# Kari-Genomics-Lab/iDeLUCS

Measured on AMD Instinct MI355X. Metric: sequences/sec (k-mer vectorise + 1 epoch), k=6 batch 512, higher is better.
Workload: dtype f32

## Files before the change

idelucs_amd/csrc/scaler_device.h:

```cpp
#pragma once
#include <hip/hip_runtime.h>
#include <stdint.h>

#include "planes.h"
#include "store_policy.h"

namespace idl_dev {

__device__ __forceinline__ float std_f32(float x, double m, double s)
{
    const float t = (float)((double)x - m);
    return (float)((double)t / s);
}

__device__ __forceinline__ float std_f32_rcp(float x, double m, double s, double r)
{
    const double t = (double)(float)((double)x - m);
    const double q = t * r;
    return (float)fma(fma(-q, s, t), r, q);
}

struct GatherArgs {
    const float *feats;
    int64_t n, f, view_stride;
    const int64_t *pair_idx;
    const int64_t *base;
    int64_t batch, n_pairs;
    const double *mean, *scale, *inv_scale;
    float *y;
    int64_t base_add;
    uint16_t *yh, *yl;
    int *over;
    int wt;
};

__device__ __forceinline__ void gather_row(const GatherArgs &g, int64_t row, int tid, int nthreads)
{
    const int64_t b = row < g.batch ? row : row - g.batch;
    const int64_t at = (g.base ? *g.base : 0) + g.base_add + b;
    if (g.n_pairs >= 0 && at >= g.n_pairs) return;
    const int64_t pair = g.pair_idx[at];
    const int64_t m = pair / g.n, s = pair - m * g.n;
    const float *src = g.feats + (row < g.batch ? 0 : (m + 1) * g.view_stride) + s * g.f;
    float *dst = g.y + row * g.f;
    if ((g.f & 3) == 0) {
        const float4 *src4 = (const float4 *)src;
        float4 *dst4 = (float4 *)dst;
        const int64_t n4 = g.f / 4;
        for (int64_t i0 = tid; i0 < n4; i0 += 4 * (int64_t)nthreads) {
            float4 vv[4];
#pragma unroll
            for (int u = 0; u < 4; ++u) {
                const int64_t i = i0 + (int64_t)u * nthreads;
                if (i < n4) vv[u] = src4[i];
            }
#pragma unroll
// ... 16 lines not shown
                }
                dst4[i] = o;
            }
        }
    } else {
        for (int64_t i = tid; i < g.f; i += nthreads) dst[i] = std_f32(src[i], g.mean[i], g.scale[i]);
    }
}

constexpr int GATHER_ROWS = 8;

__host__ __device__ inline int64_t gather_blocks(int64_t f, int64_t batch)
{
    if (f & 3) return 2 * batch;
    return ((2 * batch + GATHER_ROWS - 1) / GATHER_ROWS) * ((f / 4 + 255) / 256);
}

template <int R>
__host__ __device__ inline int64_t gather_tiles(int64_t f, int64_t batch)
{
    return ((2 * batch + R - 1) / R) * ((f / 4 + 255) / 256);
}

template <int R>
__device__ __forceinline__ void gather_tile(const GatherArgs &g, int64_t blk, int tid)
{
    const int64_t n4 = g.f / 4, slices = (n4 + 255) / 256;
    const int64_t rg = blk / slices, i = (blk - rg * slices) * 256 + tid;
    if (i >= n4) return;
    const int64_t base = (g.base ? *g.base : 0) + g.base_add;
    const bool wt = (g.wt & idl_store::WT_NEXT_PLANES) != 0;
    const bool paired = wt && (n4 & 1) == 0 && ((((uintptr_t)g.yh) | ((uintptr_t)g.yl)) & 15u) == 0;
    const float4 *src4[R];
    float4 vv[R];
#pragma unroll
    for (int u = 0; u < R; ++u) {
        const int64_t row = rg * R + u;
        const int64_t b = row < g.batch ? row : row - g.batch;
        const int64_t at = base + b;
        src4[u] = nullptr;
        if (row < 2 * g.batch && (g.n_pairs < 0 || at < g.n_pairs)) {
            const int64_t pair = g.pair_idx[at];
            const int64_t m = pair / g.n, s = pair - m * g.n;
            src4[u] = (const float4 *)(g.feats + (row < g.batch ? 0 : (m + 1) * g.view_stride) + s * g.f);
        }
    }
#pragma unroll
    for (int u = 0; u < R; ++u)
        if (src4[u] != nullptr) vv[u] = src4[u][i];
    const int64_t c = i * 4;
    double mu[4], sc[4], rc[4];
#pragma unroll
    for (int e = 0; e < 4; ++e) { mu[e] = g.mean[c + e]; sc[e] = g.scale[c + e]; rc[e] = g.inv_scale ? g.inv_scale[c + e] : 0.0; }
#pragma unroll
    for (int u = 0; u < R; ++u) {
        if (src4[u] == nullptr) continue;
        const float4 v = vv[u];
        float4 o;
        if (g.inv_scale != nullptr) {
            o.x = std_f32_rcp(v.x, mu[0], sc[0], rc[0]); o.y = std_f32_rcp(v.y, mu[1], sc[1], rc[1]);
            o.z = std_f32_rcp(v.z, mu[2], sc[2], rc[2]); o.w = std_f32_rcp(v.w, mu[3], sc[3], rc[3]);
        } else {
            o.x = std_f32(v.x, mu[0], sc[0]); o.y = std_f32(v.y, mu[1], sc[1]);
            o.z = std_f32(v.z, mu[2], sc[2]); o.w = std_f32(v.w, mu[3], sc[3]);
        }
        if (g.y != nullptr) idl_store::store16((float4 *)(g.y + (rg * R + u) * g.f) + i, o, wt);
        if (g.yh != nullptr) {
            constexpr float ps = (float)(1 << idl_planes::X_EXP);
            uint2 h, l;
            if (idl_planes::split4(o.x * ps, o.y * ps, o.z * ps, o.w * ps, h, l) && g.over != nullptr) *g.over = 1;
            if (paired) {
                const bool odd = (tid & 1) != 0;
                idl_store::store16_wt((uint2 *)((odd ? g.yl : g.yh) + (rg * R + u) * g.f) + (i - (odd ? 1 : 0)), idl_store::pair_planes(h, l, odd));
            } else {
                ((uint2 *)(g.yh + (rg * R + u) * g.f))[i] = h;
                ((uint2 *)(g.yl + (rg * R + u) * g.f))[i] = l;
            }
        }
    }
}

__device__ __forceinline__ void gather_block(const GatherArgs &g, int64_t blk, int tid)
{
    if (g.f & 3) { gather_row(g, blk, tid, 256); return; }
    gather_tile<GATHER_ROWS>(g, blk, tid);
}

}
```

idelucs_amd/csrc/train_step.hip:

```cpp
#include <stdlib.h>
#include "dev_env.h"
#include <string.h>

#include "common.h"
#include "iic_device.h"
#include "nce_device.h"
#include "scaler_device.h"
#include "wave_ops.h"
#include "wgrad_device.h"
#include "l1_device.h"
#include "l1_planes_device.h"
#include "wgrad_planes_device.h"
#include "mid_fwd_device.h"

namespace {

using mid_dev::H1;
using mid_dev::H2;
using mid_dev::MAX_CPL;
using mid_dev::f32x4_t;
constexpr int COL_PARTS = 64;


#ifdef IDL_PHASE_STAMPS
// ... 30 lines not shown
        if (c < C) {
            float acc = b3[c];
            const float *wr = W3 + (int64_t)c * H2;
#pragma unroll 8
            for (int h = 0; h < H2; ++h) acc = fmaf(sh[h], wr[h], acc);
            lg.v[t] = acc;
        }
    }
    mid_dev::softmax_row(lg, row, lane, C, true, z);
    __builtin_amdgcn_wave_barrier();
}

__global__ __launch_bounds__(256) void head_fwd_kernel(const float *lat, const float *W3, const float *b3, int m, int C, int train,
                                                       uint64_t seed, const int64_t *ctl, float *f, float *inv, float *r2, float *z)
{
    __shared__ float sh[4][H2];
    const int w = threadIdx.x >> 6, lane = threadIdx.x & 63;
    const int row = blockIdx.x * 4 + w;
    if (row >= m) return;
    head_row(lat[(int64_t)row * H2 + lane], row, lane, sh[w], W3, b3, C, train, seed, (uint32_t)ctl[0], f, inv, r2, z);
}

constexpr int MID_WAVES = mid_dev::WAVES;
constexpr int MID_GATHER_ROWS = 4;

template <bool TIN>
__device__ __forceinline__ void mid_fwd_body(float *__restrict__ a1, const float *__restrict__ b1, const float *__restrict__ W2,
                                                                  const float *__restrict__ b2, const float *__restrict__ W3,
                                                                  const float *__restrict__ b3, int m, int C, int train, uint64_t seed,
                                                                  const int64_t *__restrict__ ctl, float *__restrict__ f,
                                                                  float *__restrict__ inv, float *__restrict__ r2, float *__restrict__ z,
                                                                  int n_rows_wg, int tile0, int tile1, const idl_dev::GatherArgs &gth, const int bid)
{
    if (bid >= n_rows_wg) {
        const int blk = tile0 + (bid - n_rows_wg) * 4 + (int)(threadIdx.x >> 8);
        if (blk < tile1) idl_dev::gather_tile<MID_GATHER_ROWS>(gth, (int64_t)blk, (int)(threadIdx.x & 255));
        return;
    }
    __shared__ float part[MID_WAVES][16][H2];
    float (*R2t)[H2 + 4] = (float (*)[H2 + 4])&part[0][0][0];
    float (*LG)[64 * MAX_CPL + 1] = (float (*)[64 * MAX_CPL + 1])&part[2][0][0];
    const int lane = threadIdx.x & 63, wv = threadIdx.x >> 6, l = lane & 15, q = lane >> 4;
    const int r0 = bid * 16;
    uint64_t *stf = IDL_PHASE_BUF(1, bid);
    IDL_PHASE_STAMP(stf, 0);
    const int k0 = 32 * wv + 8 * q;
    float4 *src = (float4 *)(a1 + (int64_t)(r0 + l) * H1 + k0);
    float *srcT = a1 + (int64_t)k0 * m + r0 + l;
    float4 av[2] = {make_float4(0.f, 0.f, 0.f, 0.f), make_float4(0.f, 0.f, 0.f, 0.f)};
    float4 bb[2] = {make_float4(0.f, 0.f, 0.f, 0.f), make_float4(0.f, 0.f, 0.f, 0.f)};
    mid_dev::W2Tile bw[4];
    auto load_bw = [&]() {
#pragma unroll
        for (int ct = 0; ct < 4; ++ct) bw[ct] = mid_dev::load_w2(W2, ct, l, k0);
    };
    float t8[8] = {0.f, 0.f, 0.f, 0.f, 0.f, 0.f, 0.f, 0.f};
    if (TIN) {
#pragma unroll
        for (int i = 0; i < 8; ++i) t8[i] = srcT[(int64_t)i * m];
        av[0] = make_float4(t8[0], t8[1], t8[2], t8[3]); av[1] = make_float4(t8[4], t8[5], t8[6], t8[7]);
    } else {
        av[0] = src[0]; av[1] = src[1];
// ... 328 lines not shown
            acc += v;
        }
    }
    sh[w][lane] = acc;
    __syncthreads();
    if (w == 0 && c < n) job.partial[(int64_t)blockIdx.y * n + c] = (sh[0][lane] + sh[1][lane]) + (sh[2][lane] + sh[3][lane]);
}

struct MidBwdArgs {
    const float *z, *r2, *f, *inv, *G, *dP0, *W3, *W2, *act1;
    float *dlogits, *dlat, *dr1, *partial1, *partial2, *partial3, *dW3_part;
    int64_t *ctl; int64_t batch_advance;
    int g_parts, m, C, train; float nce_coef;
    int act1_t;
    uint16_t *dr1h, *dr1l;
    int *dscale, *dover;
    const float *dzs;
};

template <bool BIG = false, bool DP = false>
__device__ __forceinline__ void mid_bwd_body(const MidBwdArgs &a, int tile0, int tile1, const idl_dev::GatherArgs &gth, const int bid)
{
    extern __shared__ float mid_dyn[];
    if (bid >= COL_PARTS) {
        const int blk = tile0 + (bid - COL_PARTS) * 4 + (int)(threadIdx.x >> 8);
        if (blk < tile1) idl_dev::gather_tile<MID_GATHER_ROWS>(gth, (int64_t)blk, (int)(threadIdx.x & 255));
        return;
    }
    __shared__ float DL[16][H2 + 4];
    __shared__ float R2s[16][H2];
    __shared__ float DLG[16][64 * MAX_CPL];
    __shared__ float shz[MID_WAVES][64 * MAX_CPL];
    __shared__ float sP[48 * 48], sW3[48 * H2];
    const int lane = threadIdx.x & 63, wv = threadIdx.x >> 6, l = lane & 15, q = lane >> 4, tid = threadIdx.x;
    const int m = a.m, C = a.C, B = m / 2;
    constexpr bool small = !BIG;
    const int rows = (m + COL_PARTS - 1) / COL_PARTS;
    const int r0 = bid * rows;
    const int r1 = (r0 + rows < m) ? r0 + rows : m;
    uint64_t *stb = IDL_PHASE_BUF(2, bid);
    IDL_PHASE_STAMP(stb, 0);
    if (a.ctl != nullptr && bid == 0 && tid == 0) a.ctl[1] += a.batch_advance;
    __shared__ unsigned int s_dmx, s_dcnt;
    const int dk = DP ? a.dscale[1] : 0;
    if (DP && tid == 0) { s_dmx = 0u; s_dcnt = 0u; }
    unsigned int dmx = 0u;
    if (small) {
        for (int i = tid; i < C * C; i += 64 * MID_WAVES) sP[i] = a.dP0[i];
        for (int i = tid; i < C * H2; i += 64 * MID_WAVES) sW3[i] = a.W3[i];
    } else {
        for (int i = tid; i < C * H2; i += 64 * MID_WAVES) mid_dyn[i] = a.W3[i];
    }
    float bw[2][16];
#pragma unroll
    for (int s = 0; s < 16; ++s) {
// ... 209 lines not shown
    }
    if (te < H2) a.partial2[(int64_t)bid * H2 + te] = s23;
    else if (te < H2 + C) a.partial3[(int64_t)bid * C + te - H2] = s23;
    if (a.dW3_part != nullptr) {
#pragma unroll
        for (int i = 0; i < 3; ++i) {
            const int o = te + 1024 * i;
            if (o < C * H2) a.dW3_part[(int64_t)bid * C * H2 + o] = acc3[i];
        }
    }
    IDL_PHASE_STAMP(stb, 6);
}
struct MidBwdParams { MidBwdArgs a; int tile0, tile1; idl_dev::GatherArgs gth; };
static_assert(sizeof(MidBwdParams) + idl::PLAN_PARAMS <= idl::PLAN_BYTES, "MidBwdParams does not fit a plan record");

template <bool BIG = false, bool DP = false>
__global__ __launch_bounds__(64 * MID_WAVES) void mid_bwd_kernel(MidBwdArgs a, int tile0, int tile1, idl_dev::GatherArgs gth)
{
    mid_bwd_body<BIG, DP>(a, tile0, tile1, gth, (int)blockIdx.x);
}

__global__ __launch_bounds__(64 * MID_WAVES) void mid_bwd_batched_kernel(const unsigned char *__restrict__ plans)
{
    const MidBwdParams &p = *(const MidBwdParams *)(plans + (size_t)blockIdx.x * idl::PLAN_BYTES + idl::PLAN_PARAMS);
    if (p.a.dr1h != nullptr) mid_bwd_body<false, true>(p.a, p.tile0, p.tile1, p.gth, (int)blockIdx.y);
    else mid_bwd_body<false, false>(p.a, p.tile0, p.tile1, p.gth, (int)blockIdx.y);
}

__global__ __launch_bounds__(64 * MID_WAVES) void mid_bwd_big_batched_kernel(const unsigned char *__restrict__ plans)
{
    const MidBwdParams &p = *(const MidBwdParams *)(plans + (size_t)blockIdx.x * idl::PLAN_BYTES + idl::PLAN_PARAMS);
    mid_bwd_body<true, true>(p.a, p.tile0, p.tile1, p.gth, (int)blockIdx.y);
}

struct RmsArgs {
    const float *loss_rows;
    float *out;
    int loss_m;
    float w_nce, w_iic;
    float *p[8];
    const float *g[8];
    float *v[8];
    int64_t n[8];
    int parts[8];
    int count;
    const float *wg_dy, *wg_x; float *wg_grad;
// ... 232 lines not shown
#pragma unroll
        for (int u = 0; u < RED_U; ++u) {
            const int64_t i = i0 + 256 * u < r.slab4 ? i0 + 256 * u : r.slab4 - 1;
#pragma unroll
            for (int p = 0; p < l1p_dev::KSPLIT; ++p) v[u][p] = r.part[(int64_t)p * r.slab4 + i];
        }
#pragma unroll
        for (int u = 0; u < RED_U; ++u) {
            float4 acc = v[u][0];
#pragma unroll
            for (int p = 1; p < l1p_dev::KSPLIT; ++p) { acc.x += v[u][p].x; acc.y += v[u][p].y; acc.z += v[u][p].z; acc.w += v[u][p].w; }
            if (i0 + 256 * u < r.slab4) r.part[i0 + 256 * u] = acc;
        }
        return;
    }
    if (with_tail) rmsprop_body<true>(a, hyper, ctl, batch_advance, 0, 0, idl_dev::GatherArgs{}, (int)blockIdx.x, (int)threadIdx.x);
}

struct SumsFwdArgs {
    const float *b1, *W2, *b2, *W3, *b3; float *r1T; int m, C, train; uint64_t seed; float *f, *inv, *r2, *z; int tile0, tile1; idl_dev::GatherArgs gth;
};
constexpr int SUMS_FWD_ROWS = 8;
constexpr int SUMS_FWD_LDS = (MID_WAVES * SUMS_FWD_ROWS * H2 + 16 * (H2 + 4) + SUMS_FWD_ROWS * (64 * MAX_CPL + 1)) * (int)sizeof(float);

__device__ __forceinline__ void sums_fwd_body(const ReduceArgs &r, const SumsFwdArgs &p, float *smem, const int bid)
{
    constexpr int ROWS = SUMS_FWD_ROWS, GROUPS = 16 / ROWS, SPL = l1p_dev::KSPLIT / GROUPS, Q0 = 4 - ROWS / 4;
    if (bid >= r.blocks) {
        const int blk = p.tile0 + (bid - r.blocks) * 4 + (int)(threadIdx.x >> 8);
        if (blk < p.tile1) idl_dev::gather_tile<MID_GATHER_ROWS>(p.gth, (int64_t)blk, (int)(threadIdx.x & 255));
        return;
    }
    float (*ps)[ROWS][H2] = (float (*)[ROWS][H2])smem;
    float (*R2t)[H2 + 4] = (float (*)[H2 + 4])(smem + MID_WAVES * ROWS * H2);
    float (*LG)[64 * MAX_CPL + 1] = (float (*)[64 * MAX_CPL + 1])(smem + MID_WAVES * ROWS * H2 + 16 * (H2 + 4));
    const int lane = threadIdx.x & 63, wv = threadIdx.x >> 6, l = lane & 15, q = lane >> 4;
    const int grp = l / ROWS, rr = l % ROWS;
    const bool own = grp == GROUPS - 1;
    const int m = p.m, C = p.C, train = p.train;
    const int r0 = bid * ROWS;
    const int k0 = 32 * wv + 8 * q;
    const int64_t e4 = ((int64_t)(r0 + rr) * H1 + k0) / 4;
    float4 pv[SPL][2];
#pragma unroll
    for (int j = 0; j < SPL; ++j) {
        const float4 *src = r.part + (int64_t)(SPL * grp + j) * r.slab4 + e4;
        pv[j][0] = src[0]; pv[j][1] = src[1];
    }
    float4 bb[2];
    bb[0] = *(const float4 *)(p.b1 + k0); bb[1] = *(const float4 *)(p.b1 + k0 + 4);
    mid_dev::W2Tile bw[4];
#pragma unroll
    for (int ct = 0; ct < 4; ++ct) bw[ct] = mid_dev::load_w2(p.W2, ct, l, k0);
// ... 195 lines not shown
                 float *f, float *inv, float *r2, float *z, void *stream)
{
    IDL_REQUIRE(lat && W3 && b3 && ctl && f && inv && r2 && z, "NULL buffer");
    IDL_REQUIRE(m >= 1 && C >= 1 && C <= 64 * MAX_CPL, "head_fwd: n_clusters must be in 1..256");
    hipLaunchKernelGGL(head_fwd_kernel, dim3((unsigned)((m + 3) / 4)), dim3(256), 0, (hipStream_t)stream, lat, W3, b3, m, C, train, seed,
                       ctl, f, inv, r2, z);
    IDL_HIP_TRY(hipGetLastError());
    return IDL_OK;
}

int idl_mid_fwd(float *a1, const float *W2, const float *b2, const float *W3, const float *b3, int m, int C, int train,
                uint64_t seed, const int64_t *ctl, float *f, float *inv, float *r2, float *z, void *stream)
{
    IDL_REQUIRE(a1 && W2 && b2 && W3 && b3 && ctl && f && inv && r2 && z, "NULL buffer");
    IDL_REQUIRE(m >= 16 && (m % 16) == 0 && C >= 1 && C <= 64 * MAX_CPL, "mid_fwd: m must be a multiple of 16, n_clusters in 1..256");
    IDL_REQUIRE((((uintptr_t)a1 | (uintptr_t)W2 | (uintptr_t)W3) & 15u) == 0, "a1 / W2 / W3 must be 16-byte aligned");
    hipLaunchKernelGGL(mid_fwd_kernel<false>, dim3((unsigned)(m / 16)), dim3(64 * MID_WAVES), 0, (hipStream_t)stream, a1, (const float *)nullptr, W2, b2,
                       W3, b3, m, C, train, seed, ctl, f, inv, r2, z, m / 16, 0, 0, idl_dev::GatherArgs{});
    IDL_HIP_TRY(hipGetLastError());
    return IDL_OK;
}

struct Riders {
    idl_dev::GatherArgs g{}; int t0 = 0, t1 = 0;
    unsigned wgs() const { return (unsigned)((t1 - t0 + 3) / 4); }
};
static int riders_of(const char *who, const idl_next_batch_t *nb, Riders &out)
{
    const auto bad = [who](const char *what) { idl::set_error("bad argument: %s: %s", who, what); return IDL_ERR_ARG; };
    out = Riders{};
    if (nb == nullptr) return IDL_OK;
    uint16_t *yh = (uint16_t *)nb->y_hi, *yl = (uint16_t *)nb->y_lo;
    if (!(nb->parts >= 1 && nb->part >= 0 && nb->part <= nb->part_end && nb->part_end <= nb->parts)) return bad("need 0 <= part <= part_end <= parts");
    if (!((yh != nullptr) == (yl != nullptr) && (yh == nullptr || (nb->feats != nullptr && ((((uintptr_t)yh) | ((uintptr_t)yl)) & 7u) == 0))))
        return bad("both planes of the next batch (8-byte aligned) or neither; planes need the batch assembly");
    if (nb->feats == nullptr) return IDL_OK;
    if (!(nb->pair_idx && nb->mean && nb->scale && (nb->y || yh) && nb->n >= 1 && nb->f >= 4 && (nb->f & 3) == 0 && nb->batch >= 1 && nb->n_pairs >= 0))
        return bad("bad gather arguments (4 | f)");
    out.g = idl_dev::GatherArgs{nb->feats, nb->n, nb->f, nb->view_stride, nb->pair_idx, nb->base, nb->batch, nb->n_pairs, nb->mean, nb->scale, nb->inv_scale, nb->y,
                                nb->base_add, yh, yl, nb->overflow_flag, idl_store::wt_mask()};
    const int64_t ng = idl_dev::gather_tiles<MID_GATHER_ROWS>(nb->f, nb->batch);
    out.t0 = (int)(ng * nb->part / nb->parts); out.t1 = (int)(ng * nb->part_end / nb->parts);
    return IDL_OK;
}

int idl_mid_fwd_gather(float *a1, const float *b1, int a1_transposed, const float *W2, const float *b2, const float *W3, const float *b3, int m,
                       int C, int train, uint64_t seed, const int64_t *ctl, float *f, float *inv, float *r2, float *z,
                       const idl_next_batch_t *next_batch, void *stream)
{
    IDL_REQUIRE(a1 && W2 && b2 && W3 && b3 && ctl && f && inv && r2 && z, "NULL buffer");
    IDL_REQUIRE(m >= 16 && (m % 16) == 0 && C >= 1 && C <= 64 * MAX_CPL, "mid_fwd: m must be a multiple of 16, n_clusters in 1..256");
    IDL_REQUIRE((((uintptr_t)a1 | (uintptr_t)W2 | (uintptr_t)W3) & 15u) == 0, "a1 / W2 / W3 must be 16-byte aligned");
    IDL_REQUIRE(b1 == nullptr || (((uintptr_t)b1) & 15u) == 0, "mid_fwd_gather: b1 must be 16-byte aligned");
    IDL_REQUIRE(a1_transposed == 0 || a1_transposed == 1, "mid_fwd_gather: a1_transposed is 0 or 1");
    Riders rd;
    if (const int rc = riders_of("mid_fwd_gather", next_batch, rd)) return rc;
    const dim3 grid((unsigned)(m / 16) + rd.wgs());
    if (void *plan = idl::take_plan()) {
        idl::fill_plan(plan, idl::PLAN_MID_FWD, a1_transposed , grid, 64 * MID_WAVES, 0,
                       MidFwdParams{a1, b1, W2, b2, W3, b3, m, C, train, seed, ctl, f, inv, r2, z, m / 16, rd.t0, rd.t1, rd.g});
        return IDL_OK;
    }
    if (a1_transposed) hipLaunchKernelGGL(mid_fwd_kernel<true>, grid, dim3(64 * MID_WAVES), 0, (hipStream_t)stream, a1, b1, W2, b2, W3, b3,
                                          m, C, train, seed, ctl, f, inv, r2, z, m / 16, rd.t0, rd.t1, rd.g);
    else hipLaunchKernelGGL(mid_fwd_kernel<false>, grid, dim3(64 * MID_WAVES), 0, (hipStream_t)stream, a1, b1, W2, b2, W3, b3,
                            m, C, train, seed, ctl, f, inv, r2, z, m / 16, rd.t0, rd.t1, rd.g);
    IDL_HIP_TRY(hipGetLastError());
    return IDL_OK;
}

int idl_nce_rows(float *S, int m, float temperature, float *lse, float *loss_rows, void *stream)
{
    IDL_REQUIRE(S && lse && loss_rows && m >= 2 && (m % 2) == 0 && temperature > 0.f, "nce_rows: even m >= 2, T > 0");
    const float inv_t = 1.f / temperature;
    hipLaunchKernelGGL(nce_lse_kernel, dim3((unsigned)((m + 3) / 4)), dim3(256), 0, (hipStream_t)stream, S, m, inv_t, lse, loss_rows);
    int64_t g = ((int64_t)m * m + 255) / 256;
    if (g > 4096) g = 4096;
    hipLaunchKernelGGL(nce_esym_kernel, dim3((unsigned)g), dim3(256), 0, (hipStream_t)stream, S, m, inv_t, lse);
    IDL_HIP_TRY(hipGetLastError());
// ... 85 lines not shown
}


int idl_mid_bwd_gather(const float *z, const float *r2, const float *f, const float *inv, const float *G, int g_parts, const float *dP0,
                       const float *W3, const float *W2, const float *act1, int m, int C, int train, float nce_coef, float *dlogits,
                       float *dlat, float *dr1, float *partial1, float *partial2, float *partial3, float *dW3_partial, int act1_transposed,
                       void *dr1_hi, void *dr1_lo, int *dr1_scale, int *dr1_overflow_flag, const float *z_dP0, const idl_next_batch_t *next_batch, void *stream)
{
    uint16_t *dr1h = (uint16_t *)dr1_hi, *dr1l = (uint16_t *)dr1_lo;
    IDL_REQUIRE((dr1h != nullptr) == (dr1l != nullptr) && (dr1h == nullptr || (dr1_scale && dr1_overflow_flag && ((((uintptr_t)dr1h) | ((uintptr_t)dr1l)) & 15u) == 0)),
                "mid_bwd_gather: dr1's planes need both planes (16-byte aligned), the words of their scale and the flag");
    IDL_REQUIRE(g_parts >= 1 && g_parts <= 16, "mid_bwd: g_parts outside 1..16");
    IDL_REQUIRE(z && r2 && f && inv && G && dP0 && W3 && W2 && act1 && dlogits && dlat && (dr1 || dr1h) && partial1 && partial2 && partial3, "NULL buffer");
    IDL_REQUIRE(m >= 2 && (m % 2) == 0 && C >= 1 && C <= 64 * MAX_CPL, "mid_bwd: even m, n_clusters in 1..256");
    IDL_REQUIRE(dW3_partial == nullptr || C <= 48, "mid_bwd: dW3 partials need n_clusters <= 48");
    MidBwdArgs a{};
    a.dr1h = dr1h; a.dr1l = dr1l; a.dscale = dr1_scale; a.dover = dr1_overflow_flag; a.dzs = z_dP0;
    IDL_REQUIRE(z_dP0 == nullptr || C > 48, "mid_bwd_gather: z dP0 as an input is the n_clusters > 48 form");
    a.z = z; a.r2 = r2; a.f = f; a.inv = inv; a.G = G; a.dP0 = dP0; a.W3 = W3; a.W2 = W2; a.act1 = act1;
    a.dlogits = dlogits; a.dlat = dlat; a.dr1 = dr1; a.partial1 = partial1; a.partial2 = partial2; a.partial3 = partial3;
    a.dW3_part = dW3_partial; a.ctl = nullptr; a.batch_advance = 0;
    a.g_parts = g_parts; a.m = m; a.C = C; a.train = train; a.nce_coef = nce_coef; a.act1_t = act1_transposed ? 1 : 0;
    Riders rd;
    if (const int rc = riders_of("mid_bwd_gather", next_batch, rd)) return rc;
    const unsigned grid = (unsigned)COL_PARTS + rd.wgs();
    if (void *plan = idl::take_plan()) {
        IDL_REQUIRE(C <= 48 || (dr1h != nullptr && z_dP0 != nullptr),
                    "mid_bwd_gather: beyond 48 classes only the form with dr1 as planes and z dP0 given can be recorded");
        idl::fill_plan(plan, idl::PLAN_MID_BWD, C > 48 ? 1 : 0, dim3(grid), 64 * MID_WAVES, C > 48 ? (unsigned)(C * H2 * (int)sizeof(float)) : 0u,
                       MidBwdParams{a, rd.t0, rd.t1, rd.g});
        return IDL_OK;
    }
    if (C > 48) return dr1h != nullptr ? launch_mid_bwd_big<true>(a, grid, rd.t0, rd.t1, rd.g, stream) : launch_mid_bwd_big<false>(a, grid, rd.t0, rd.t1, rd.g, stream);
    if (dr1h != nullptr) hipLaunchKernelGGL((mid_bwd_kernel<false, true>), dim3(grid), dim3(64 * MID_WAVES), 0, (hipStream_t)stream, a, rd.t0, rd.t1, rd.g);
    else hipLaunchKernelGGL((mid_bwd_kernel<false, false>), dim3(grid), dim3(64 * MID_WAVES), 0, (hipStream_t)stream, a, rd.t0, rd.t1, rd.g);
    IDL_HIP_TRY(hipGetLastError());
    return IDL_OK;
}

int idl_col_sum_parts(void) { return COL_PARTS; }

static int launch_col_jobs(ColJobs &jobs, int njobs, void *stream)
{
    int nb = 0;
    for (int k = 0; k < 3; ++k) {
        jobs.first_block[k] = nb;
        if (k < njobs) nb += (jobs.j[k].n + 63) / 64;
// ... 229 lines not shown
            return IDL_OK;
        }
        hipLaunchKernelGGL(reduce_rms_kernel, dim3((unsigned)r.blocks), dim3(256), 0, (hipStream_t)stream, r, RmsArgs{}, (const float *)nullptr, (int64_t *)nullptr,
                           (int64_t)0, 0);
        IDL_HIP_TRY(hipGetLastError());
        return IDL_OK;
    }
    TailCarrier by;
    by.red = &r;
    return rmsprop_launch(*tail, idl_dev::GatherArgs{}, stream, by);
}

int idl_reduce_mid_fwd_gather_planes(const float *part, const int64_t *step_counter, int64_t *step_snapshot, float *r1_transposed,
                                     const float *b1, const float *W2, const float *b2, const float *W3, const float *b3, int m,
                                     int C, int train, uint64_t seed, float *f, float *inv, float *r2, float *z,
                                     const idl_next_batch_t *next_batch, void *stream)
{
    IDL_REQUIRE(part && step_counter && r1_transposed && b1 && W2 && b2 && W3 && b3 && f && inv && r2 && z, "reduce_mid_fwd: NULL buffer");
    IDL_REQUIRE(m >= 16 && (m % 16) == 0 && C >= 1 && C <= 64 * MAX_CPL && (int64_t)m * H1 < (1ll << 31), "reduce_mid_fwd: m must be a multiple of 16, n_clusters in 1..256");
    IDL_REQUIRE((((uintptr_t)part | (uintptr_t)b1 | (uintptr_t)W2 | (uintptr_t)W3) & 15u) == 0 && (((uintptr_t)r1_transposed) & 3u) == 0,
                "reduce_mid_fwd: part / b1 / W2 / W3 must be 16-byte aligned");
    IDL_REQUIRE(idl::take_plan() == nullptr, "reduce_mid_fwd: the lone voter's launch, not recordable");
    Riders rd;
    if (const int rc = riders_of("reduce_mid_fwd", next_batch, rd)) return rc;
    const ReduceArgs r{(float4 *)const_cast<float *>(part), (int64_t)m * H1 / 4, l1p_dev::KSPLIT, m / SUMS_FWD_ROWS, step_counter, step_snapshot};
    const SumsFwdArgs p{b1, W2, b2, W3, b3, r1_transposed, m, C, train, seed, f, inv, r2, z, rd.t0, rd.t1, rd.g};
    hipLaunchKernelGGL(sums_fwd_kernel, dim3((unsigned)r.blocks + rd.wgs()), dim3(64 * MID_WAVES), SUMS_FWD_LDS, (hipStream_t)stream, r, p);
    IDL_HIP_TRY(hipGetLastError());
    return IDL_OK;
}

int idl_wgrad_xplanes_rms(const void *dy_hi, const void *dy_lo, int *dy_scale, const void *x_hi, const void *x_lo, int ld_x, int m, int n_out, int n_in, float *grad, float *W,
                          float *square_avg, void *w_hi, void *w_lo, int *overflow_flag, const idl_opt_tail_t *tail, void *stream)
{
    IDL_REQUIRE(tail != nullptr, "wgrad_xplanes_rms: NULL tail");
    const float *hyper = tail->hyper;
    IDL_REQUIRE(dy_hi && dy_lo && dy_scale && x_hi && x_lo && W && square_avg && hyper && tail->ctl && w_hi && w_lo && overflow_flag, "wgrad_xplanes_rms: NULL buffer");
    IDL_REQUIRE(idl_wgrad_xplanes_supported(m, n_out, n_in), "wgrad_xplanes_rms: m % 64 == 0, m >= 192, n_out % 64 == 0, n_in % 128 == 0");
    IDL_REQUIRE(ld_x >= n_in && ld_x <= n_in + 1024 && (ld_x & 7) == 0, "wgrad_xplanes_rms: n_in <= ld_x <= n_in + 1024, 8 | ld_x");
    IDL_REQUIRE((((uintptr_t)dy_hi | (uintptr_t)dy_lo | (uintptr_t)x_hi | (uintptr_t)x_lo | (uintptr_t)grad | (uintptr_t)W | (uintptr_t)square_avg) & 15u) == 0 &&
                (((uintptr_t)w_hi | (uintptr_t)w_lo) & 7u) == 0, "wgrad_xplanes_rms: buffers 16-byte aligned, W's planes 8-byte");
    wgp_dev::XpArgs x{};
    x.dyh = (const uint16_t *)dy_hi; x.dyl = (const uint16_t *)dy_lo; x.dy_scale = dy_scale;
    x.xh = (const uint16_t *)x_hi; x.xl = (const uint16_t *)x_lo; x.grad = grad; x.W = W; x.V = square_avg;
    x.wh = (uint16_t *)w_hi; x.wl = (uint16_t *)w_lo; x.over = overflow_flag; x.hyper = hyper;
    x.m = m; x.n_out = n_out; x.n_in = n_in; x.ldx = ld_x;
    x.tiles_m = n_out / wgp_dev::TM; x.tiles = x.tiles_m * (n_in / wgp_dev::TN);
// ... 101 lines not shown
```

idelucs_amd/fused.py:

```python
import ctypes
import os
import sys

import torch

from . import _lib
from ._lib import lib as _L

EPS = sys.float_info.epsilon
TEMPERATURE = 0.85


def _p(t):
    return ctypes.c_void_p(t.data_ptr()) if t is not None else None


_PLANES_DISABLED = False


def planes_default():
    return os.environ.get("IDELUCS_PLANES", "1") != "0" and not _PLANES_DISABLED


VARIANTS = {
    "test_cold": "0",
    "lockstep_planes": "1",
    "planes_wgrad": "1",
    "planes_tail": "wgrad",
    "sums_fwd": "1",
    "fused": "1",
}
VARIANTS.update({k: v for k, v in _lib.DEV.items() if k in VARIANTS})
STEPS_PER_GRAPH = 16
GATHER_SPLIT = 4
PLANES_MAX_ROWS = 60_000_000


def _v(name):
    return VARIANTS[name]


def disable_planes():
    global _PLANES_DISABLED
    _PLANES_DISABLED = True


def _stream():
    return ctypes.c_void_p(torch.cuda.current_stream().cuda_stream)


_DR1_FP32 = (None,) * 5


# ... 266 lines not shown
            bf._planes["valid"][0] = False
            bf._planes["x32"][0] = True

    def _full_step(self, store, bf, train=True, pipelined=False, xi=0, defer_tail=False):
        if pipelined:
            self.step_on_batch(bf, train=train, batch_advance=bf.m // 2, next_from=store, xi=xi if self._early(bf, store) else 0, defer_tail=defer_tail)
        else:
            self._gather(store, bf)
            self.step_on_batch(bf, train=train, batch_advance=bf.m // 2)


class FusedLinearTrainer(_LinearStepParts):
    def __init__(self, net, lr, weight, lamb, weight_decay=0.01, alpha=0.99, eps=1e-8, seed=0, grad_w1=None, shared_buffers=None):
        self._init_network(net, weight, lamb, seed, grad_w1, shared_buffers)
        self._rec = None
        self.square_avg = [torch.zeros_like(p) for p in self.params]
        self.hyper = torch.tensor([lr, alpha, eps, weight_decay, 1.0 - alpha], dtype=torch.float32, device=self.dev)
        self._cold = _v("test_cold") == "1"
        self._planes = planes_default()
        self._planes_lockstep = _v("lockstep_planes") != "0"
        self._planes_wgrad = _v("planes_wgrad") != "0"
        self._planes_tail_wgrad = _v("planes_tail") != "reduce"
        self._sums_fwd = _v("sums_fwd") == "1"
        self._cus = torch.cuda.get_device_properties(self.dev).multi_processor_count if self.dev.type == "cuda" else 0
        self._ctl_snap = torch.zeros(1, dtype=torch.int64, device=self.dev)
        self._w1_planes = None
        self._dr1_scale = torch.zeros(int(_L.idl_dr1_scale_words()), dtype=torch.int32, device=self.dev)
        self._dr1_scale[1:2].fill_(int(_L.idl_planes_exponent(2)))
        self._w1_planes_fresh = False
        self._keep_w1_grad = False
        self._pending = None
        n = len(self.params)
        self._vp = (ctypes.c_void_p * n)(*[v.data_ptr() for v in self.square_avg])

    def begin_voter(self, voter, keep_state=False):
        self.ctl[0:1].fill_((int(voter) & 0xFF) << 24)
        self._dr1_scale[1:2].fill_(int(_L.idl_planes_exponent(2)))
        if keep_state:
            return
        for v in self.square_avg:
            v.zero_()

    def set_lr(self, lr):
        self.hyper[0:1].fill_(float(lr))

    def _k(self, fn, *args):
# ... 89 lines not shown
        cold = self._cold and not rec
        pb = _planes_of(bf, F)
        xplanes, wide = bool(_L.idl_wgrad_xplanes_supported(m, H1, F)), _tile_per_cu(H1, F, self._cus)
        assert not rec or (xplanes and wide), "a recorded two-plane step ends with the tail on the dW1 tiles: _form must not record another shape"
        plw = xplanes and (rec or self._planes_wgrad)
        tail_on_wgrad = plw and wide and (rec or self._planes_tail_wgrad)
        if not plw:
            self._check_x32(bf, xi)
        part, x = pb["part"][xi], bf.xs[xi]
        merged = self._sums_fwd and tail_on_wgrad and not rec and self._pending is None
        r1 = _r1T_of(pb, bf, xi) if merged else part[0]
        if not rec:
            bf._l1_src = "r1T" if merged else "part"
        wh, wl, flag = self._planes_operands(bf, pb, xi)
        if cold:
            self._evict()
        self._k(_L.idl_l1_planes_rows if merged else _L.idl_l1_planes, _p(wh), _p(wl), F, _p(pb["xh"][xi]), _p(pb["xl"][xi]), F, m, H1, F, _p(part), _stream())
        nxt = dict(y=None if plw else bf.xs[1 - xi], planes=(pb["xh"][1 - xi], pb["xl"][1 - xi]), flag=flag)
        if merged:
            if cold:
                self._evict()
            head, outs = self._mid_fwd_tensors(bf, tr)
            _launch(_L.idl_reduce_mid_fwd_gather_planes, _p(part), _p(self.ctl), _p(self._ctl_snap), _p(r1), _p(self.b1), *head, *outs,
                    self._next_batch(st, m, part_end=GATHER_SPLIT, **nxt), _stream())
        else:
            if self._pending is not None and not rec:
                self._tail_launch(*self._pending, red=(part, H1 * m))
            else:
                self._reduce(part, m)
            if cold:
                self._evict()
            self._k(_L.idl_mid_fwd_gather, _p(part), _p(self.b1), 1, *self._mid_fwd_args(bf, tr), self._next_batch(st, m, part_end=GATHER_SPLIT, **nxt), _stream())
        launch_losses(self._k, bf, self.lamb, self.weight, self.out)
        self._k(_L.idl_mid_bwd_gather, *self._mid_bwd_args(bf, tr, r1, self.grads[4]), 1, *self._dr1_planes_args(pb, plw, flag),
                self._next_batch(st, m, part=GATHER_SPLIT, **nxt), _stream())
        if not rec:
            pb["valid"][1 - xi] = True
            pb["x32"][1 - xi] = not plw
        w1 = (None if rec else self._gw1(), _p(self.W1), _p(self.square_avg[0]))
        if tail_on_wgrad:
            if cold:
                self._evict()
            self._k(_L.idl_wgrad_xplanes_rms, *self._dy_planes_args(pb), _p(pb["xh"][xi]), _p(pb["xl"][xi]), F, m, H1, F, *w1, _p(wh), _p(wl), _p(flag),
                    self._tail(bf, skip=0, advance=m // 2, **self._wg(bf, r1, 1)), _stream())
            return
        if plw:
            _launch(_L.idl_wgrad_rmsprop_xplanes, *self._dy_planes_args(pb), _p(pb["xh"][xi]), _p(pb["xl"][xi]), F, m, H1, F, *w1, _p(self.hyper),
                    _p(wh), _p(wl), _p(flag), _stream())
        else:
            _launch(_L.idl_wgrad_rmsprop_planes, _p(bf.dr1), _p(x), m, H1, F, *w1, _p(self.hyper), _p(wh), _p(wl), _p(flag), _stream())
        self._leave_tail_pending(bf, xi, r1, defer_tail)

    def _step_planes_rows(self, bf, tr, st, xi):
        m, C, H1, F = bf.m, self.C, self.H1, self.F
        rec = self._rec is not None
        cold = self._cold and not rec
        pb = _planes_of(bf, F)
        part = pb["part"][xi]
# ... 360 lines not shown
```

Measured before the change: 2.001 million.

## Cap gather rider workgroups to spare CUs and loop tiles with LDS-staged constants

The next-batch gather used to launch one extra workgroup per four tiles. Those "rider" workgroups are now limited to the CUs left over after the computing workgroups, and each loops over several tile units with double-buffered row loads. Row source pointers and per-column mean/scale constants are staged in LDS that overlaps the computing arrays. The split of gather work between the fused reduce/mid-forward launch and the mid-backward launch also becomes a tunable share in sixteenths. The aim is to stop gather blocks from crowding the compute blocks and to amortise the pointer and constant loads, at the cost of more serial work per rider and extra barriers.

```diff
diff --git a/idelucs_amd/csrc/scaler_device.h b/idelucs_amd/csrc/scaler_device.h
--- a/idelucs_amd/csrc/scaler_device.h
+++ b/idelucs_amd/csrc/scaler_device.h
@@ -32,6 +32,7 @@
     uint16_t *yh, *yl;
     int *over;
     int wt;
+    int rounds;
 };
 
 __device__ __forceinline__ void gather_row(const GatherArgs &g, int64_t row, int tid, int nthreads)
@@ -94,48 +95,60 @@
     return ((2 * batch + R - 1) / R) * ((f / 4 + 255) / 256);
 }
 
-template <int R>
-__device__ __forceinline__ void gather_tile(const GatherArgs &g, int64_t blk, int tid)
-{
-    const int64_t n4 = g.f / 4, slices = (n4 + 255) / 256;
-    const int64_t rg = blk / slices, i = (blk - rg * slices) * 256 + tid;
-    if (i >= n4) return;
-    const int64_t base = (g.base ? *g.base : 0) + g.base_add;
+template <int R> struct TileRows { float4 v[R]; unsigned ok; };
+struct TileConsts { double mu[4], sc[4], rc[4]; };
+
+__device__ __forceinline__ const float4 *tile_row_src(const GatherArgs &g, int64_t row, int64_t base)
+{
+    const int64_t b = row < g.batch ? row : row - g.batch;
+    const int64_t at = base + b;
+    if (!(row < 2 * g.batch && (g.n_pairs < 0 || at < g.n_pairs))) return nullptr;
+    const int64_t pair = g.pair_idx[at];
+    const int64_t m = pair / g.n, s = pair - m * g.n;
+    return (const float4 *)(g.feats + (row < g.batch ? 0 : (m + 1) * g.view_stride) + s * g.f);
+}
+
+template <int R>
+__device__ __forceinline__ void tile_load(TileRows<R> &t, int u, const float4 *src, int64_t i)
+{
+    if (src != nullptr) { t.v[u] = src[i]; t.ok |= 1u << u; }
+}
+
+__device__ __forceinline__ TileConsts tile_consts(const GatherArgs &g, int64_t c)
+{
+    TileConsts k;
+#pragma unroll
+    for (int e = 0; e < 4; ++e) { k.mu[e] = g.mean[c + e]; k.sc[e] = g.scale[c + e]; k.rc[e] = g.inv_scale ? g.inv_scale[c + e] : 0.0; }
+    return k;
+}
+
+template <int R>
+__device__ __forceinline__ void tile_std_col(const GatherArgs &g, TileRows<R> &t, int e, double mu, double sc, double rc)
+{
+#pragma unroll
+    for (int u = 0; u < R; ++u) {
+        float &x = e == 0 ? t.v[u].x : e == 1 ? t.v[u].y : e == 2 ? t.v[u].z : t.v[u].w;
+        x = g.inv_scale != nullptr ? std_f32_rcp(x, mu, sc, rc) : std_f32(x, mu, sc);
+    }
+}
+
+template <int R>
+__device__ __forceinline__ void tile_std(const GatherArgs &g, TileRows<R> &t, const TileConsts &k)
+{
+#pragma unroll
+    for (int e = 0; e < 4; ++e) tile_std_col<R>(g, t, e, k.mu[e], k.sc[e], k.rc[e]);
+}
+
+template <int R>
+__device__ __forceinline__ void tile_store(const GatherArgs &g, int64_t rg, int64_t i, int tid, const TileRows<R> &t)
+{
+    const int64_t n4 = g.f / 4;
     const bool wt = (g.wt & idl_store::WT_NEXT_PLANES) != 0;
     const bool paired = wt && (n4 & 1) == 0 && ((((uintptr_t)g.yh) | ((uintptr_t)g.yl)) & 15u) == 0;
-    const float4 *src4[R];
-    float4 vv[R];
 #pragma unroll
     for (int u = 0; u < R; ++u) {
-        const int64_t row = rg * R + u;
-        const int64_t b = row < g.batch ? row : row - g.batch;
-        const int64_t at = base + b;
-        src4[u] = nullptr;
-        if (row < 2 * g.batch && (g.n_pairs < 0 || at < g.n_pairs)) {
-            const int64_t pair = g.pair_idx[at];
-            const int64_t m = pair / g.n, s = pair - m * g.n;
-            src4[u] = (const float4 *)(g.feats + (row < g.batch ? 0 : (m + 1) * g.view_stride) + s * g.f);
-        }
-    }
-#pragma unroll
-    for (int u = 0; u < R; ++u)
-        if (src4[u] != nullptr) vv[u] = src4[u][i];
-    const int64_t c = i * 4;
-    double mu[4], sc[4], rc[4];
-#pragma unroll
-    for (int e = 0; e < 4; ++e) { mu[e] = g.mean[c + e]; sc[e] = g.scale[c + e]; rc[e] = g.inv_scale ? g.inv_scale[c + e] : 0.0; }
-#pragma unroll
-    for (int u = 0; u < R; ++u) {
-        if (src4[u] == nullptr) continue;
-        const float4 v = vv[u];
-        float4 o;
-        if (g.inv_scale != nullptr) {
-            o.x = std_f32_rcp(v.x, mu[0], sc[0], rc[0]); o.y = std_f32_rcp(v.y, mu[1], sc[1], rc[1]);
-            o.z = std_f32_rcp(v.z, mu[2], sc[2], rc[2]); o.w = std_f32_rcp(v.w, mu[3], sc[3], rc[3]);
-        } else {
-            o.x = std_f32(v.x, mu[0], sc[0]); o.y = std_f32(v.y, mu[1], sc[1]);
-            o.z = std_f32(v.z, mu[2], sc[2]); o.w = std_f32(v.w, mu[3], sc[3]);
-        }
+        if ((t.ok & (1u << u)) == 0) continue;
+        const float4 o = t.v[u];
         if (g.y != nullptr) idl_store::store16((float4 *)(g.y + (rg * R + u) * g.f) + i, o, wt);
         if (g.yh != nullptr) {
             constexpr float ps = (float)(1 << idl_planes::X_EXP);
@@ -152,6 +165,86 @@
     }
 }
 
+template <int R>
+__device__ __forceinline__ void gather_tile(const GatherArgs &g, int64_t blk, int tid)
+{
+    const int64_t n4 = g.f / 4, slices = (n4 + 255) / 256;
+    const int64_t rg = blk / slices, i = (blk - rg * slices) * 256 + tid;
+    if (i >= n4) return;
+    const int64_t base = (g.base ? *g.base : 0) + g.base_add;
+    TileRows<R> t;
+    t.ok = 0u;
+    const float4 *src[R];
+#pragma unroll
+    for (int u = 0; u < R; ++u) src[u] = tile_row_src(g, rg * R + u, base);
+#pragma unroll
+    for (int u = 0; u < R; ++u) tile_load(t, u, src[u], i);
+    const TileConsts k = tile_consts(g, i * 4);
+    tile_std<R>(g, t, k);
+    tile_store<R>(g, rg, i, tid, t);
+}
+
+constexpr int RIDER_ROWS = 4;
+constexpr int RIDER_MAX_ROUNDS = 64;
+struct RiderLds { double *mu, *sc, *rc; uint64_t *rows; };
+
+__host__ __device__ inline int64_t rider_tiles(int64_t f, int64_t batch)
+{
+    const int64_t groups = (2 * batch + RIDER_ROWS - 1) / RIDER_ROWS;
+    return ((groups + 3) / 4) * ((f / 4 + 255) / 256) * 4;
+}
+
+__device__ __forceinline__ void ride(const GatherArgs &g, int t0, int t1, int w, const RiderLds &L)
+{
+    constexpr int R = RIDER_ROWS;
+    const int rounds = g.rounds;
+    const int u0 = t0 / 4 + w * rounds, u1 = min(u0 + rounds, (t1 + 3) / 4);
+    if (u0 >= u1) return;
+    const int t = (int)threadIdx.x, sub = t >> 8, tid = t & 255;
+    const int64_t n4 = g.f / 4;
+    const int quads = (int)(((2 * g.batch + R - 1) / R + 3) / 4);
+    int slice = u0 / quads;
+    double cm = 0.0, cs = 1.0, cr = 0.0;
+    auto fetch_consts = [&](int sl) {
+        const int64_t c = (int64_t)sl * 1024 + t;
+        if (c < g.f) { cm = g.mean[c]; cs = g.scale[c]; cr = g.inv_scale ? g.inv_scale[c] : 0.0; }
+    };
+    auto stage_consts = [&]() { L.mu[t] = cm; L.sc[t] = cs; L.rc[t] = cr; };
+    fetch_consts(slice);
+    if (t < (u1 - u0) * 16) {
+        const int u = u0 + (t >> 4), tile = 4 * u + ((t >> 2) & 3);
+        const int64_t row = (int64_t)(u % quads) * 16 + (t & 15);
+        const float4 *src = nullptr;
+        if (tile >= t0 && tile < t1) src = tile_row_src(g, row, (g.base ? *g.base : 0) + g.base_add);
+        L.rows[t] = (uint64_t)(uintptr_t)src;
+    }
+    stage_consts();
+    __syncthreads();
+    auto rows_of = [&](int u, TileRows<R> &tr) {
+        const int64_t i = (int64_t)(u / quads) * 256 + tid;
+        tr.ok = 0u;
+#pragma unroll
+        for (int e = 0; e < R; ++e) tile_load(tr, e, i < n4 ? (const float4 *)(uintptr_t)L.rows[(u - u0) * 16 + sub * R + e] : nullptr, i);
+    };
+    TileRows<R> cur, nxt;
+    rows_of(u0, cur);
+    for (int u = u0; u < u1; ++u) {
+        const int sl = u / quads;
+        if (u + 1 < u1) rows_of(u + 1, nxt);
+        if (sl != slice) {
+            slice = sl;
+            fetch_consts(sl);
+            __syncthreads();
+            stage_consts();
+            __syncthreads();
+        }
+#pragma unroll
+        for (int e = 0; e < 4; ++e) tile_std_col<R>(g, cur, e, L.mu[4 * tid + e], L.sc[4 * tid + e], L.rc[4 * tid + e]);
+        tile_store<R>(g, (int64_t)(u - sl * quads) * 4 + sub, (int64_t)sl * 256 + tid, tid, cur);
+        if (u + 1 < u1) cur = nxt;
+    }
+}
+
 __device__ __forceinline__ void gather_block(const GatherArgs &g, int64_t blk, int tid)
 {
     if (g.f & 3) { gather_row(g, blk, tid, 256); return; }
diff --git a/idelucs_amd/csrc/train_step.hip b/idelucs_amd/csrc/train_step.hip
--- a/idelucs_amd/csrc/train_step.hip
+++ b/idelucs_amd/csrc/train_step.hip
@@ -76,7 +76,12 @@
 }
 
 constexpr int MID_WAVES = mid_dev::WAVES;
-constexpr int MID_GATHER_ROWS = 4;
+constexpr int RIDER_LDS_BYTES = 3 * 1024 * (int)sizeof(double) + idl_dev::RIDER_MAX_ROUNDS * 16 * (int)sizeof(uint64_t);
+__device__ __forceinline__ idl_dev::RiderLds rider_lds(float *at)
+{
+    double *d = (double *)at;
+    return idl_dev::RiderLds{d, d + 1024, d + 2048, (uint64_t *)(d + 3072)};
+}
 
 template <bool TIN>
 __device__ __forceinline__ void mid_fwd_body(float *__restrict__ a1, const float *__restrict__ b1, const float *__restrict__ W2,
@@ -86,12 +91,11 @@
                                                                   float *__restrict__ inv, float *__restrict__ r2, float *__restrict__ z,
                                                                   int n_rows_wg, int tile0, int tile1, const idl_dev::GatherArgs &gth, const int bid)
 {
+    __shared__ __attribute__((aligned(16))) float part[MID_WAVES][16][H2];
     if (bid >= n_rows_wg) {
-        const int blk = tile0 + (bid - n_rows_wg) * 4 + (int)(threadIdx.x >> 8);
-        if (blk < tile1) idl_dev::gather_tile<MID_GATHER_ROWS>(gth, (int64_t)blk, (int)(threadIdx.x & 255));
+        idl_dev::ride(gth, tile0, tile1, bid - n_rows_wg, rider_lds(&part[0][0][0]));
         return;
     }
-    __shared__ float part[MID_WAVES][16][H2];
     float (*R2t)[H2 + 4] = (float (*)[H2 + 4])&part[0][0][0];
     float (*LG)[64 * MAX_CPL + 1] = (float (*)[64 * MAX_CPL + 1])&part[2][0][0];
     const int lane = threadIdx.x & 63, wv = threadIdx.x >> 6, l = lane & 15, q = lane >> 4;
@@ -466,15 +470,15 @@
 __device__ __forceinline__ void mid_bwd_body(const MidBwdArgs &a, int tile0, int tile1, const idl_dev::GatherArgs &gth, const int bid)
 {
     extern __shared__ float mid_dyn[];
-    if (bid >= COL_PARTS) {
-        const int blk = tile0 + (bid - COL_PARTS) * 4 + (int)(threadIdx.x >> 8);
-        if (blk < tile1) idl_dev::gather_tile<MID_GATHER_ROWS>(gth, (int64_t)blk, (int)(threadIdx.x & 255));
-        return;
-    }
     __shared__ float DL[16][H2 + 4];
     __shared__ float R2s[16][H2];
-    __shared__ float DLG[16][64 * MAX_CPL];
-    __shared__ float shz[MID_WAVES][64 * MAX_CPL];
+    __shared__ __attribute__((aligned(16))) float DLG[16][64 * MAX_CPL];
+    __shared__ __attribute__((aligned(16))) float shz[MID_WAVES][64 * MAX_CPL];
+    if (bid >= COL_PARTS) {
+        double *d0 = (double *)&DLG[0][0], *d1 = (double *)&shz[0][0];
+        idl_dev::ride(gth, tile0, tile1, bid - COL_PARTS, idl_dev::RiderLds{d0, d0 + 1024, d1, (uint64_t *)(d1 + 1024)});
+        return;
+    }
     __shared__ float sP[48 * 48], sW3[48 * H2];
     const int lane = threadIdx.x & 63, wv = threadIdx.x >> 6, l = lane & 15, q = lane >> 4, tid = threadIdx.x;
     const int m = a.m, C = a.C, B = m / 2;
@@ -730,6 +734,7 @@
 
 __global__ __launch_bounds__(64 * MID_WAVES) void mid_bwd_batched_kernel(const unsigned char *__restrict__ plans)
 {
+    asm volatile("" ::: "v127");
     const MidBwdParams &p = *(const MidBwdParams *)(plans + (size_t)blockIdx.x * idl::PLAN_BYTES + idl::PLAN_PARAMS);
     if (p.a.dr1h != nullptr) mid_bwd_body<false, true>(p.a, p.tile0, p.tile1, p.gth, (int)blockIdx.y);
     else mid_bwd_body<false, false>(p.a, p.tile0, p.tile1, p.gth, (int)blockIdx.y);
@@ -1008,13 +1013,14 @@
 };
 constexpr int SUMS_FWD_ROWS = 8;
 constexpr int SUMS_FWD_LDS = (MID_WAVES * SUMS_FWD_ROWS * H2 + 16 * (H2 + 4) + SUMS_FWD_ROWS * (64 * MAX_CPL + 1)) * (int)sizeof(float);
+static_assert(RIDER_LDS_BYTES <= SUMS_FWD_LDS && RIDER_LDS_BYTES <= (int)sizeof(float) * MID_WAVES * 16 * H2 && RIDER_LDS_BYTES == 2 * 16 * 64 * MAX_CPL * (int)sizeof(float),
+              "the riders' LDS lies over the computing workgroups' arrays");
 
 __device__ __forceinline__ void sums_fwd_body(const ReduceArgs &r, const SumsFwdArgs &p, float *smem, const int bid)
 {
     constexpr int ROWS = SUMS_FWD_ROWS, GROUPS = 16 / ROWS, SPL = l1p_dev::KSPLIT / GROUPS, Q0 = 4 - ROWS / 4;
     if (bid >= r.blocks) {
-        const int blk = p.tile0 + (bid - r.blocks) * 4 + (int)(threadIdx.x >> 8);
-        if (blk < p.tile1) idl_dev::gather_tile<MID_GATHER_ROWS>(p.gth, (int64_t)blk, (int)(threadIdx.x & 255));
+        idl_dev::ride(p.gth, p.tile0, p.tile1, bid - r.blocks, rider_lds(smem));
         return;
     }
     float (*ps)[ROWS][H2] = (float (*)[ROWS][H2])smem;
@@ -1256,10 +1262,10 @@
 }
 
 struct Riders {
-    idl_dev::GatherArgs g{}; int t0 = 0, t1 = 0;
-    unsigned wgs() const { return (unsigned)((t1 - t0 + 3) / 4); }
+    idl_dev::GatherArgs g{}; int t0 = 0, t1 = 0, n = 0;
+    unsigned wgs() const { return (unsigned)n; }
 };
-static int riders_of(const char *who, const idl_next_batch_t *nb, Riders &out)
+static int riders_of(const char *who, const idl_next_batch_t *nb, int computing_wgs, Riders &out)
 {
     const auto bad = [who](const char *what) { idl::set_error("bad argument: %s: %s", who, what); return IDL_ERR_ARG; };
     out = Riders{};
@@ -1273,8 +1279,23 @@
         return bad("bad gather arguments (4 | f)");
     out.g = idl_dev::GatherArgs{nb->feats, nb->n, nb->f, nb->view_stride, nb->pair_idx, nb->base, nb->batch, nb->n_pairs, nb->mean, nb->scale, nb->inv_scale, nb->y,
                                 nb->base_add, yh, yl, nb->overflow_flag, idl_store::wt_mask()};
-    const int64_t ng = idl_dev::gather_tiles<MID_GATHER_ROWS>(nb->f, nb->batch);
+    const int64_t ng = idl_dev::rider_tiles(nb->f, nb->batch);
+    if (!(ng < (1ll << 30))) return bad("too many tiles");
     out.t0 = (int)(ng * nb->part / nb->parts); out.t1 = (int)(ng * nb->part_end / nb->parts);
+    if (out.t1 <= out.t0) return IDL_OK;
+    const int units = (out.t1 + 3) / 4 - out.t0 / 4;
+    int cap = 0;
+    if (const char *e = idl::dev_env("riders_max")) cap = atoi(e);
+    if (cap < 1) {
+        idl::DeviceInfo di;
+        if (const int rc = idl::device_info(&di); rc != IDL_OK) return rc;
+        cap = di.cus - computing_wgs;
+    }
+    const int n = units < cap ? units : (cap < 1 ? 1 : cap);
+    int rounds = (units + n - 1) / n;
+    if (rounds > idl_dev::RIDER_MAX_ROUNDS) rounds = idl_dev::RIDER_MAX_ROUNDS;
+    out.n = (units + rounds - 1) / rounds;
+    out.g.rounds = rounds;
     return IDL_OK;
 }
 
@@ -1288,7 +1309,7 @@
     IDL_REQUIRE(b1 == nullptr || (((uintptr_t)b1) & 15u) == 0, "mid_fwd_gather: b1 must be 16-byte aligned");
     IDL_REQUIRE(a1_transposed == 0 || a1_transposed == 1, "mid_fwd_gather: a1_transposed is 0 or 1");
     Riders rd;
-    if (const int rc = riders_of("mid_fwd_gather", next_batch, rd)) return rc;
+    if (const int rc = riders_of("mid_fwd_gather", next_batch, m / 16, rd)) return rc;
     const dim3 grid((unsigned)(m / 16) + rd.wgs());
     if (void *plan = idl::take_plan()) {
         idl::fill_plan(plan, idl::PLAN_MID_FWD, a1_transposed , grid, 64 * MID_WAVES, 0,
@@ -1420,7 +1441,7 @@
     a.dW3_part = dW3_partial; a.ctl = nullptr; a.batch_advance = 0;
     a.g_parts = g_parts; a.m = m; a.C = C; a.train = train; a.nce_coef = nce_coef; a.act1_t = act1_transposed ? 1 : 0;
     Riders rd;
-    if (const int rc = riders_of("mid_bwd_gather", next_batch, rd)) return rc;
+    if (const int rc = riders_of("mid_bwd_gather", next_batch, COL_PARTS, rd)) return rc;
     const unsigned grid = (unsigned)COL_PARTS + rd.wgs();
     if (void *plan = idl::take_plan()) {
         IDL_REQUIRE(C <= 48 || (dr1h != nullptr && z_dP0 != nullptr),
@@ -1696,7 +1717,7 @@
                 "reduce_mid_fwd: part / b1 / W2 / W3 must be 16-byte aligned");
     IDL_REQUIRE(idl::take_plan() == nullptr, "reduce_mid_fwd: the lone voter's launch, not recordable");
     Riders rd;
-    if (const int rc = riders_of("reduce_mid_fwd", next_batch, rd)) return rc;
+    if (const int rc = riders_of("reduce_mid_fwd", next_batch, m / SUMS_FWD_ROWS, rd)) return rc;
     const ReduceArgs r{(float4 *)const_cast<float *>(part), (int64_t)m * H1 / 4, l1p_dev::KSPLIT, m / SUMS_FWD_ROWS, step_counter, step_snapshot};
     const SumsFwdArgs p{b1, W2, b2, W3, b3, r1_transposed, m, C, train, seed, f, inv, r2, z, rd.t0, rd.t1, rd.g};
     hipLaunchKernelGGL(sums_fwd_kernel, dim3((unsigned)r.blocks + rd.wgs()), dim3(64 * MID_WAVES), SUMS_FWD_LDS, (hipStream_t)stream, r, p);
diff --git a/idelucs_amd/fused.py b/idelucs_amd/fused.py
--- a/idelucs_amd/fused.py
+++ b/idelucs_amd/fused.py
@@ -29,6 +29,7 @@
     "planes_tail": "wgrad",
     "sums_fwd": "1",
     "fused": "1",
+    "rider_share": "8",
 }
 VARIANTS.update({k: v for k, v in _lib.DEV.items() if k in VARIANTS})
 STEPS_PER_GRAPH = 16
@@ -341,6 +342,9 @@
         self._planes_wgrad = _v("planes_wgrad") != "0"
         self._planes_tail_wgrad = _v("planes_tail") != "reduce"
         self._sums_fwd = _v("sums_fwd") == "1"
+        self._rider_share = int(_v("rider_share"))
+        if not 0 <= self._rider_share <= 16:
+            raise ValueError("VARIANTS['rider_share'] counts sixteenths: 0..16")
         self._cus = torch.cuda.get_device_properties(self.dev).multi_processor_count if self.dev.type == "cuda" else 0
         self._ctl_snap = torch.zeros(1, dtype=torch.int64, device=self.dev)
         self._w1_planes = None
@@ -476,7 +480,7 @@
                 self._evict()
             head, outs = self._mid_fwd_tensors(bf, tr)
             _launch(_L.idl_reduce_mid_fwd_gather_planes, _p(part), _p(self.ctl), _p(self._ctl_snap), _p(r1), _p(self.b1), *head, *outs,
-                    self._next_batch(st, m, part_end=GATHER_SPLIT, **nxt), _stream())
+                    self._next_batch(st, m, part_end=self._rider_share, parts=16, **nxt), _stream())
         else:
             if self._pending is not None and not rec:
                 self._tail_launch(*self._pending, red=(part, H1 * m))
@@ -486,8 +490,9 @@
                 self._evict()
             self._k(_L.idl_mid_fwd_gather, _p(part), _p(self.b1), 1, *self._mid_fwd_args(bf, tr), self._next_batch(st, m, part_end=GATHER_SPLIT, **nxt), _stream())
         launch_losses(self._k, bf, self.lamb, self.weight, self.out)
-        self._k(_L.idl_mid_bwd_gather, *self._mid_bwd_args(bf, tr, r1, self.grads[4]), 1, *self._dr1_planes_args(pb, plw, flag),
-                self._next_batch(st, m, part=GATHER_SPLIT, **nxt), _stream())
+        rest = self._next_batch(st, m, part=GATHER_SPLIT, **nxt) if not merged else \
+            self._next_batch(st, m, part=self._rider_share, part_end=16, parts=16, **nxt) if self._rider_share < 16 else None
+        self._k(_L.idl_mid_bwd_gather, *self._mid_bwd_args(bf, tr, r1, self.grads[4]), 1, *self._dr1_planes_args(pb, plw, flag), rest, _stream())
         if not rec:
             pb["valid"][1 - xi] = True
             pb["x32"][1 - xi] = not plw
```

Result: slower. 1.978 million (-1.2%).
